# YxZhxn/Ray3D

Hardware: AMD Instinct MI355X
Metric: lifted poses/sec (17-joint, 243-frame window) (higher is better)
Workload: dtype f32; 1 GPU; BASELINE configs[1]: synthetic 17-joint 243-frame windows, batch 256 per GPU, forward-only pos+trj (C=256, latent 256, stage 3, camera embedding); batch_per_gpu=256, receptive_field=243, joints=17, parallelism=dp1 (independent window batches, no data-path collective), clock_settle_steps=60, world_size_observed=1

## Files before the change

### ray3d_amd/csrc/r3d_forward.cpp

```cpp
#include <algorithm>
#include <cstring>
#include <mutex>

#include "r3d_internal.hpp"
#include "r3d_undistort.hpp"

namespace r3d {

static void output_slots(int J, const int *first, int *slot) {
    int s = 0;
    auto put = [&](int part, int idx) {
        for (int f = 0; f < 3; ++f) slot[first[part] + idx * 3 + f] = s * 3 + f;
        ++s;
    };
    enum { T = 0, LA = 1, RA = 2, LL = 3, RL = 4 };
    if (J == 17) {
        put(T, 0);
        for (int i = 0; i < 3; ++i) put(LL, i);
        for (int i = 0; i < 3; ++i) put(RL, i);
        for (int i = 1; i < 5; ++i) put(T, i);
        for (int i = 0; i < 3; ++i) put(RA, i);
        for (int i = 0; i < 3; ++i) put(LA, i);
    } else if (J == 15) {
        put(T, 0); put(T, 1);
// ... 347 lines not shown
    hipError_t e;
    if ((e = c.rec.begin("r3d_event_pair", -1, 0, 0.0, 0.0)) != hipSuccess) return hip_fail(e, "hipEventRecord");
    if ((e = c.rec.end()) != hipSuccess) return hip_fail(e, "hipEventRecord");
    return R3D_OK;
}

int px_prepass(Call &c) {
    if (!c.in_px) return R3D_OK;
    const Model *a = c.a;
    const r3d_input *in_px = c.in_px;
    UndistArgs ua;
    memset(&ua, 0, sizeof ua);
    ua.uv = in_px->x_dev;
    ua.cam = in_px->cam_dev;
    ua.cam_stride = in_px->cam_stride;
    ua.rays = const_cast<float *>(c.in->x_dev);
    ua.J = a->cfg.num_joints;
    ua.npts = (int)(dist_ray_frames(a, in_px, c.B) * a->cfg.num_joints);
    ua.pts_per_window = dist_materialised(a, in_px) ? a->RF * a->cfg.num_joints : 0;
    ua.window_stride = (int)in_px->window_stride;
    ua.last_window = (int)(c.B - 1);
    ua.encoding = px_encoding(in_px->mode);
    if (const int rc = c.begin("r3d_undistort_rays_f64", (ua.npts + 255) / 256, 0.0, (double)ua.npts * (2 + enc_floats(ua.encoding)) * sizeof(float)); rc != R3D_OK)
        return rc;
    if (const hipError_t e = launch_undistort(ua, c.stream); e != hipSuccess) return hip_fail(e, "launch r3d_undistort_rays_f64");
    return c.end();
}

int pick_schedule(Call &c) {
    const Model *a = c.a, *b = c.b;
    const r3d_input *in = c.in;
    const Plan *pl = c.pl;
    c.uv = in->mode == R3D_INPUT_UV;
    c.JF = frame_floats(a, c.uv);
    c.bases.ws = reinterpret_cast<const char *>(c.ws);
    for (int mi = 0; mi < 2; ++mi)
        if (pl->m[mi]) {
            c.bases.arena[mi] = reinterpret_cast<const char *>(pl->m[mi]->d_arena);
            c.bases.iarena[mi] = reinterpret_cast<const char *>(pl->m[mi]->d_iarena);
        }
    c.bases.x = reinterpret_cast<const char *>(in->x_dev);
    c.bases.param = reinterpret_cast<const char *>(in->param_dev);
    c.bases.cam = reinterpret_cast<const char *>(in->cam_dev);
    c.shape.uv = c.uv;
    c.shape.window_stride = in->window_stride;
    c.shape.param_stride = in->param_stride;
    c.shape.cam_stride = in->cam_stride;
    c.shape.frames = c.frames;

    const FwdKeys keys = forward_keys(a, b);
    c.cu_limit = keys.cu_limit;
    c.sched = schedule_get(c.pl, c.B, keys.nwg, false, keys.lane_key0 + c.lane);
    if (!c.sched) return R3D_ERR_HIP;
    const Schedule *sched = c.sched;
    bool b3_call = false;
    for (const Model *mm : pl->m) b3_call = b3_call || (mm && mm->use_b3 && c.B >= b3_min_batch());
    c.shared = pl->frame_buf >= 0 && sched->d_frame_tiles != nullptr && in->window_stride == 1 && !b3_call &&
               (c.frames - 2) * 4 <= c.B * (int64_t)(a->RF / 3) && !(c.uv && in->cam_stride != 0) && !hook_on("R3D_NO_SHARED_L0") &&
               (unsigned long long)c.frames * (unsigned long long)pl->frame_ld * 4ull < 0xffffffffull;
    c.shape.shared = c.shared;
    c.variant = (c.uv ? 1 : 0) + (c.shared ? 2 : 0);
    c.single = forward_single_launch() && !a->opt_staged && !(b && b->opt_staged) && sched->fwd.grid > 0 && sched->fwd.d_rel[c.variant] != nullptr &&
               !(c.shared && sched->fwd.kernel != FWD_KERNEL_F32);
    return R3D_OK;
}

int frame_stage(Call &c) {
    if (!c.shared) return R3D_OK;
    const Plan *pl = c.pl;
    const r3d_input *in = c.in;
    const bool uv = c.uv;
    const StageSchedule &fs = c.sched->frame_stage;
    LaunchArgs la;
    memset(&la, 0, sizeof la);
    la.tiles = c.sched->d_frame_tiles;
    la.wg_off = c.sched->d_frame_wgoff;
    la.nprob = (int)pl->frame_probs.size();
    la.ks = fs.ks;
    float *fbase = reinterpret_cast<float *>(c.ws) + (size_t)pl->buffers[pl->frame_buf].offset_per_window * (size_t)c.B;
    for (int i = 0; i < la.nprob; ++i) {
        const Plan::FrameProb &f = pl->frame_probs[i];
        const Model *mm = pl->m[f.model];
        const Layer &L = mm->layers[f.layer];
        GemmProb &g = la.p[i];
        for (int sg = 0; sg < MAX_SEG; ++sg) g.kend[sg] = 0x7fffffff;
        g.w = mm->d_arena + L.w_off;
        g.bias = mm->d_arena + L.b_off;
        g.c = fbase + f.col;
        g.ldc = pl->frame_ld;
        g.M = (int)(c.frames - 2);
        g.N = L.N;
        g.K = L.Kpad;
        g.slope = 1.0f;
        g.lut = mm->d_iarena + (uv ? f.lut_uv : f.lut);
        g.x = reinterpret_cast<const float *>(in->x_dev);
        g.cam = uv ? reinterpret_cast<const double *>(in->cam_dev) : nullptr;
        g.cam_stride = 0;
        g.enc_ws = 0;
        g.enc_rows = g.M;
        g.enc_step = 1;
        g.enc_jf = c.JF;
        g.enc_cur = 0;
        g.enc_bytes = (unsigned)((size_t)c.frames * c.JF * sizeof(float));
        g.res_tap = 1;
    }
    if (const int rc = c.begin(uv ? "r3d_gemm_uv_f32" : "r3d_gemm_f32", fs.nwg, 0.0, 0.0); rc != R3D_OK) return rc;
    if (const hipError_t e = launch_gemm_stage(la, fs.nwg, STAGE_BIG, uv, c.stream); e != hipSuccess)
        return hip_fail(e, "launch r3d_gemm_f32 (per-frame first layers)");
    return c.end();
}


struct Single {
    hipStreamCaptureStatus cap = hipStreamCaptureStatusNone;
    bool own = false;
    bool poll = false;
    bool bound = false;
    char *ctrl = nullptr;
    size_t bank_bytes = 0;
    GemmProb *tables = nullptr;
    int bank = 0;
    unsigned *cnt = nullptr;
    BoundKey key;
};

void resolve_single(const Call &c, Single &s) {
    const Schedule::Fwd &fw = c.sched->fwd;
    const r3d_input *in = c.in;
    if (hipStreamIsCapturing(c.stream, &s.cap) != hipSuccess) { (void)hipGetLastError(); s.cap = hipStreamCaptureStatusActive; }
    s.own = s.cap == hipStreamCaptureStatusNone && fw.d_ctrl != nullptr;
    s.ctrl = s.own ? fw.d_ctrl : reinterpret_cast<char *>(c.ws) + workspace_act_bytes(c.pl, c.B);
    s.bank_bytes = ((size_t)(fw.ncnt + 4) * sizeof(unsigned) + 255) / 256 * 256;
    s.tables = reinterpret_cast<GemmProb *>(s.ctrl + (s.own ? 2 : 1) * s.bank_bytes);
    s.poll = s.own && fw.d_act != nullptr;
    s.key.variant = c.variant;
    s.key.base[BIND_WS] = c.ws;
    s.key.base[BIND_ARENA0] = c.bases.arena[0];
    s.key.base[BIND_ARENA1] = c.bases.arena[1];
    s.key.base[BIND_IARENA0] = c.bases.iarena[0];
    s.key.base[BIND_IARENA1] = c.bases.iarena[1];
    s.key.base[BIND_X] = in->x_dev;
    s.key.base[BIND_PARAM] = in->param_dev;
    s.key.base[BIND_CAM] = in->cam_dev;
    s.key.enc_ws = in->window_stride * c.JF;
    s.key.cam_stride = in->cam_stride;
    s.key.enc_bytes = (unsigned)((size_t)c.frames * c.JF * sizeof(float));
    s.key.param_stride = (int)in->param_stride;
    const Schedule::Fwd::Bound &bd = fw.bound;
    s.bound = s.own && bd.valid && bd.key == s.key;
    s.bank = s.bound ? bd.bank ^ 1 : 0;
    s.cnt = reinterpret_cast<unsigned *>(s.ctrl + (s.own ? s.bank : 0) * s.bank_bytes);
}

int bind_if_needed(Call &c, const Single &s) {
    if (s.bound) return R3D_OK;
    const Schedule::Fwd &fw = c.sched->fwd;
    BindArgs ba;
    memset(&ba, 0, sizeof ba);
    ba.rel = fw.d_rel[c.variant];
    ba.tags = fw.d_tags[c.variant];
    ba.out = s.tables;
    ba.nprob = fw.nprob;
    for (int k = 0; k < BIND_NBASE; ++k) ba.base[k] = s.key.base[k];
    ba.enc_ws = s.key.enc_ws;
    ba.cam_stride = s.key.cam_stride;
    ba.enc_bytes = s.key.enc_bytes;
    ba.param_stride = s.key.param_stride;
    ba.cnt = reinterpret_cast<unsigned *>(s.ctrl);
    ba.ncnt = s.own ? (int)(2 * s.bank_bytes / sizeof(unsigned)) - 4 : fw.ncnt;
    if (s.poll) {
        ba.base[BIND_WS] = fw.d_act;
        ba.arm = fw.d_act;
        ba.canon = 1;
        ba.arm_vec4 = (long long)(2 * fw.act_bytes / 16);
    }
    hipError_t e;
    if (const int rc = c.begin("r3d_bind_f32", 1, 0.0, 0.0); rc != R3D_OK) return rc;
    if ((e = launch_bind(ba, c.stream)) != hipSuccess) return hip_fail(e, "launch r3d_bind_f32");
    if (s.poll) {
        BindArgs b1 = ba;
        b1.base[BIND_WS] = fw.d_act + fw.act_bytes;
        b1.out = s.tables + fw.nprob;
        b1.ncnt = -4;
        b1.arm = nullptr;
        if ((e = launch_bind(b1, c.stream)) != hipSuccess) return hip_fail(e, "launch r3d_bind_f32");
    }
    return c.end();
}

int launch_tiles(Call &c, const Single &s, FwdArgs &fa) {
    Schedule::Fwd &fw = c.sched->fwd;
    const GemmProb *table = s.tables + (s.poll ? s.bank * fw.nprob : 0);
    if (s.poll) c.act_base = reinterpret_cast<float *>(fw.d_act + (size_t)s.bank * fw.act_bytes);
    fw.bound.valid = false;
    memset(&fa, 0, sizeof fa);
    fa.tiles = fw.d_tiles;
    fa.wg_off = fw.d_wgoff;
    fa.probs = table;
    fa.cnt = s.cnt;
    fa.cnt_next = s.own ? reinterpret_cast<unsigned *>(s.ctrl + (s.bank ^ 1) * s.bank_bytes) : nullptr;
    fa.ncnt = fw.ncnt;
    if (s.poll) {
        fa.poll = 1;
        fa.arm = fw.d_act + (size_t)(s.bank ^ 1) * fw.act_bytes;
        fa.arm_vec4 = (long long)(fw.act_bytes / 16);
    }
    fa.spin_ticks = (long long)std::max(c.a->spin_timeout_ms, 1) * 100000LL;
    if (const char *ft = hook_env("R3D_FAULT_TILE")) fa.fault_tile1 = atoi(ft) + 1;
    const bool uv_launch = c.uv && fw.uses_gather;
    const int fwd_kernel = c.shared ? FWD_KERNEL_CLIP : fw.kernel;
    if (const int rc = c.begin(forward_kernel_name(fwd_kernel, uv_launch), fw.grid, fw.flops, fw.bytes); rc != R3D_OK) return rc;
#ifdef R3D_TIMING
    timing_arm_forward(fw, fa, c.stream);
#endif
    if (const hipError_t e = launch_forward(fa, fw.grid, fwd_kernel, uv_launch, c.stream); e != hipSuccess) return hip_fail(e, "launch r3d_forward_f32");
    c.a->last_clk_dev = s.cap == hipStreamCaptureStatusNone ? s.cnt + fw.ncnt + 2 : nullptr;
    return R3D_OK;
}

int launch_in_order(Call &c, const Single &s, FwdArgs &fa) {
    Model *a = c.a;
    hipError_t e;
    std::lock_guard<std::mutex> launch_lock(g_fwd_launch_mu);
    if ((e = order_single_launch(c.stream, true, c.cu_limit > 0)) != hipSuccess) return hip_fail(e, "hipStreamWaitEvent");
    if (c.cu_limit > 0 && a->lanes <= 1 && a->last_fwd_stream && a->last_fwd_stream != c.stream) {
        if ((e = wait_behind(c.stream, (hipStream_t)a->last_fwd_stream, a->order_ev)) != hipSuccess) return hip_fail(e, "hipStreamWaitEvent");
    }
    a->last_fwd_stream = c.stream;
    if (const int rc = bind_if_needed(c, s); rc != R3D_OK) return rc;
    if (const int rc = launch_tiles(c, s, fa); rc != R3D_OK) return rc;
    if ((e = order_single_launch(c.stream, false, c.cu_limit > 0)) != hipSuccess) return hip_fail(e, "hipEventRecord");
    return R3D_OK;
}

int single_launch(Call &c) {
    Schedule::Fwd &fw = c.sched->fwd;
    Single s;
    resolve_single(c, s);
    FwdArgs fa;
    if (const int rc = launch_in_order(c, s, fa); rc != R3D_OK) return rc;
    if (s.own) {
        fw.bound.valid = true;
        fw.bound.bank = s.bank;
        fw.bound.key = s.key;
    }
#ifdef R3D_TIMING
    timing_report_forward(c.pl, fw, fa, c.B, c.stream);
#endif
    if (const int rc = c.end(); rc != R3D_OK) return rc;
    c.abort_flag = s.cnt + fw.ncnt;
    return R3D_OK;
}

int staged_level(Call &c, size_t si) {
    const Plan *pl = c.pl;
    const auto &st = (*c.sched->levels)[si];
    const StageSchedule &ss = c.sched->stages[si];
    LaunchArgs la;
    memset(&la, 0, sizeof la);
    la.tiles = c.sched->d_tiles + ss.tiles_off;
    la.wg_off = c.sched->d_wgoff + ss.wgoff_off;
    la.nprob = (int)st.size();
    la.ks = ss.ks;
    int n_enc = 0;
    for (int i = 0; i < la.nprob; ++i) {
        const ProbSpec &q = pl->probs[st[i] & ~STAGE_SPILL_IN];
        if (q.enc_lut >= 0 && q.enc_kernel) ++n_enc;
        const int rc = fill_prob(pl, q, c.B, c.a, c.bases, c.shape, la.p[i], nullptr);
        if (rc != R3D_OK) return rc;
    }
    if (n_enc != 0 && n_enc != la.nprob) { set_error("internal: launch mixes encoded and plain operands"); return R3D_ERR_STATE; }
    if ((n_enc != 0) != (ss.kind == STAGE_ENC)) { set_error("internal: schedule and plan disagree on the launch kind"); return R3D_ERR_STATE; }
    bool uv_launch = false;
    for (int i = 0; i < la.nprob; ++i) uv_launch = uv_launch || la.p[i].cam != nullptr;
    bool b3_launch = false;
    for (int i = 0; i < la.nprob; ++i) b3_launch = b3_launch || la.p[i].wb3 != nullptr;
    const char *kname = ss.kind == STAGE_ENC ? (uv_launch ? "r3d_gemm_enc_uv_f32" : "r3d_gemm_enc_f32")
                      : b3_launch ? (uv_launch ? "r3d_gemm_uv_b3" : "r3d_gemm_b3") : (uv_launch ? "r3d_gemm_uv_f32" : "r3d_gemm_f32");
    if (const int rc = c.begin(kname, ss.nwg, ss.flops, ss.bytes); rc != R3D_OK) return rc;
#ifdef R3D_TIMING
    const bool timed = timing_arm_stage(si, la, c.stream);
#endif
    if (const hipError_t e = launch_gemm_stage(la, ss.nwg, ss.kind, uv_launch, c.stream); e != hipSuccess) return hip_fail(e, "launch r3d_gemm_f32");
#ifdef R3D_TIMING
    if (timed) timing_report_stage(si, ss, c.stream);
#endif
    return c.end();
}

int staged_levels(Call &c) {
    c.a->last_clk_dev = nullptr;
    for (size_t si = 0; si < c.sched->levels->size(); ++si)
        if (const int rc = staged_level(c, si); rc != R3D_OK) return rc;
    return R3D_OK;
}

int decoder_tail(Call &c) {
    const Model *a = c.a;
    const Plan *pl = c.pl;
    auto buf_ptr = [&](int id) -> float * { return c.act_base + (size_t)pl->buffers[id].offset_per_window * (size_t)c.B; };
    DecodeArgs da;
    memset(&da, 0, sizeof da);
    da.B = c.B;
    da.J = a->cfg.num_joints;
    da.has_pos = pl->pos_model >= 0;
    da.has_trj = pl->trj_model >= 0;
    da.out = c.out;
    da.out_trj = da.has_pos ? c.out_trj : nullptr;
    da.abort_flag = c.abort_flag;
    da.status = a->status_host;
    double dec_flops = 0;
    int first = 0;
    std::vector<Plan::Dec> order;
    for (const auto &d : pl->decs) if (pl->m[d.model]->cfg.kind == R3D_KIND_POS) order.push_back(d);
    for (const auto &d : pl->decs) if (pl->m[d.model]->cfg.kind == R3D_KIND_TRJ) order.push_back(d);
    int firsts[MAX_DEC] = {0};
    for (const auto &d : order) {
        const Model *m = pl->m[d.model];
        const Layer &L = m->layers[d.layer];
        const int sidx = da.nsrc++;
        da.h[sidx] = buf_ptr(d.hbuf);
        da.w[sidx] = m->d_arena + L.w_off;
        da.bias[sidx] = m->d_arena + L.b_off;
        da.n_out[sidx] = L.N;
        da.first[sidx] = first;
        firsts[sidx] = first;
        if (m->cfg.kind == R3D_KIND_POS) first += L.N;
        dec_flops += 2.0 * (double)c.B * L.K * L.N;
    }
    if (da.has_pos) output_slots(da.J, firsts, da.slot);
    if (const int rc = c.begin(c.B >= 128 ? "r3d_decode_w4_f32" : "r3d_decode_f32", 0, dec_flops, (double)c.B * da.nsrc * MLP_HIDDEN * 4.0); rc != R3D_OK) return rc;
    if (const hipError_t e = launch_decode(da, c.stream); e != hipSuccess) return hip_fail(e, "launch r3d_decode_f32");
    if (const int rc = c.end(); rc != R3D_OK) return rc;
    if (c.rec.on()) c.a->nrec = (int)c.rec.n;
    return R3D_OK;
}

int relay_done(Call &c) {
    Model::Lane *relay = c.relay;
    if (!relay) return R3D_OK;
    if (const hipError_t e = hipEventRecord(relay->done, relay->stream); e != hipSuccess) return hip_fail(e, "hipEventRecord(lane)");
    if (std::find(relay->waiters.begin(), relay->waiters.end(), c.caller_stream) == relay->waiters.end()) relay->waiters.push_back(c.caller_stream);
    return R3D_OK;
}

}

int forward_run(Model *a, Model *b, const r3d_input *in, int64_t B, float *out, float *out_trj, void *ws, size_t ws_bytes,
                void *stream) {
    Call c{a, b, in, B, out, out_trj, ws, ws_bytes, stream, (hipStream_t)stream};
    int rc = check_call(c);
    if (rc == R3D_OK) rc = redirect_px(c);
    if (rc == R3D_OK) rc = pick_plan(c);
    if (rc == R3D_OK) rc = pick_lane(c);
    if (rc == R3D_OK) rc = empty_bracket(c);
    if (rc == R3D_OK) rc = px_prepass(c);
    if (rc == R3D_OK) rc = pick_schedule(c);
    if (rc == R3D_OK) rc = frame_stage(c);
    if (rc == R3D_OK) rc = c.single ? single_launch(c) : staged_levels(c);
    if (rc == R3D_OK) rc = decoder_tail(c);
    if (rc == R3D_OK) rc = relay_done(c);
    return rc;
}

}
```

### ray3d_amd/csrc/r3d_internal.hpp

```cpp
#pragma once

#include <hip/hip_runtime.h>

#include <cstdint>
#include <cstdlib>
#include <map>
#include <mutex>
#include <string>
#include <vector>

#include "ray3d_hip.h"

namespace r3d {

constexpr int BK = 32;
constexpr int MAX_SEG = 4;
constexpr int MAX_PROB = 12;
constexpr int N_ALIGN = 256;
constexpr int MLP_HIDDEN = 1024;
constexpr int EMBED_MID = 32;
constexpr int CUR_LD = 64;


struct GemmProb {
    const float *a[MAX_SEG];
    int lda[MAX_SEG];
    int kend[MAX_SEG];
    const float *w;
    const float *bias;
    const float *res;
    float *c;
    int ldr, ldc;
    int M, N, K;
    float slope;
    const float *w2;
    const float *bias2;
    int K2;
    float slope2;
    const float *wb3;
    const float *w2b3, *w3b3;
    const float *w3;
    const float *bias3;
    int K3;
    float slope3;
    const int *lut;
    const float *x;
    long long enc_ws;
    int enc_rows;
    int enc_jf;
    int enc_cur;
    int enc_step;
    unsigned enc_bytes;
    int res_tap;
    int canon;
    const double *cam;
    long long cam_stride;
};

struct LaunchArgs {
    const int4 *tiles;
    const int *wg_off;
    int nprob;
    int ks;
    long long *dbg;
    GemmProb p[MAX_PROB];
};

constexpr int FWD_TILE_INT4 = 6;
constexpr int FWD_MAX_DEP = 8;
struct FwdArgs {
    const int4 *tiles;
    const int *wg_off;
    const GemmProb *probs;
    unsigned *cnt;
    unsigned *cnt_next;
    int ncnt;
    int poll;
    void *arm;
    long long arm_vec4;
    long long spin_ticks;
    int fault_tile1;
    long long *dbg;
};
enum { FWD_KERNEL_F32 = 0, FWD_KERNEL_B3 = 1, FWD_KERNEL_LAT = 2, FWD_KERNEL_CLIP = 3, FWD_KERNEL_COUNT = 4 };
constexpr int BIND_NPTR = 18;
enum { BIND_NULL = 0, BIND_WS, BIND_ARENA0, BIND_ARENA1, BIND_IARENA0, BIND_IARENA1, BIND_X, BIND_PARAM, BIND_CAM, BIND_NBASE };
struct BindArgs {
    const GemmProb *rel;
    const unsigned char *tags;
    GemmProb *out;
    unsigned *cnt;
    int nprob, ncnt;
    const void *base[BIND_NBASE];
    long long enc_ws, cam_stride;
    unsigned enc_bytes;
    int param_stride;
    int canon;
    void *arm;
    long long arm_vec4;
};

struct UndistArgs {
    const float *uv;
    const double *cam;
    long long cam_stride;
    float *rays;
    int npts;
    int J;
    int pts_per_window;
    int window_stride;
    int last_window;
    int encoding;
};

struct ClipsEncArgs {
    const r3d_clip_input_desc *table;
    const float *px;
    float *x;
    float *x_mirror;
    int32_t *status;
    long long total_frames, out_rows, max_rows;
    unsigned long long mirror_inv[2];
    int J;
    int encoding;
};

constexpr int MAX_DEC = 6;
struct DecodeArgs {
    const float *h[MAX_DEC];
    const float *w[MAX_DEC];
    const float *bias[MAX_DEC];
    int n_out[MAX_DEC];
    int first[MAX_DEC];
    int nsrc;
    int has_pos, has_trj;
    int J;
    long long B;
    float *out;
    float *out_trj;
    const unsigned *abort_flag;
    unsigned *status;
    int slot[5 * 16];
};


struct TensorSpec {
    std::string key;
    int rank;
    int64_t shape[4];
    int64_t numel() const {
        int64_t n = 1;
        for (int i = 0; i < rank; ++i) n *= shape[i];
        return n;
    }
};

inline int64_t b3_min_batch() {
    return 96;
}

inline bool env_on(const char *name) {
    const char *e = getenv(name);
    return e && atoi(e) != 0;
}
#ifdef R3D_TEST_HOOKS
inline bool hook_on(const char *name) { return env_on(name); }
inline const char *hook_env(const char *name) { return getenv(name); }
#else
inline bool hook_on(const char *) { return false; }
inline const char *hook_env(const char *) { return nullptr; }
#endif

struct Layer {
    std::string weight_key;
    std::string bias_key;
    std::string bn_prefix;
    int taps;
    int cin;
    int N, K, Npad, Kpad;
    float slope;
    std::vector<int> colmap;
    std::vector<int> colmap_neg;
    bool frag;
    size_t w_off, b_off;
    bool bf3 = false;
    bool bf3_conv = false;
    size_t wb3_off = 0;
    struct Pre { int ref_col0, ref_width, new_width, shrink_layer; };
    std::vector<Pre> pre;
    int cin_ref = 0;
    int shared_of = -1;
    int shared_split = 0;
};

struct Model {
    r3d_config cfg;
    int RF;
    std::vector<TensorSpec> specs;
    std::map<std::string, int> spec_index;
    std::vector<std::vector<float>> host_weights;
    std::vector<bool> have;
    std::vector<Layer> layers;
    std::map<std::string, int> layer_index;
    struct Branch {
        std::string prefix;
        std::vector<int> joints;
        int cin, k0, k0pad;
        size_t lut_off;
        size_t lut_uv_off;
        size_t lut_frame_off = 0, lut_frame_uv_off = 0;
        int frame_layer = -1;
    };
    std::vector<Branch> branches;
    size_t global_lut_off = 0;
    size_t global_lut_uv_off = 0;
    bool use_b3 = false;
    bool fold_shrink = false;
    std::vector<float> arena;
    std::vector<int> iarena;
    float *d_arena = nullptr;
    int *d_iarena = nullptr;
    int device = -1;
    bool finalized = false;
    bool dirty = true;
    bool opt_staged = false;
    int spin_timeout_ms = 1000;
    int cu_limit = 0;
    void *last_fwd_stream = nullptr;
    hipEvent_t order_ev = nullptr;
    int lanes = 0;
    struct Lane {
        hipStream_t stream = nullptr;
        hipEvent_t done = nullptr, in = nullptr;
        std::vector<void *> waiters;
    };
    Lane lane[4];
    int next_lane = 0;
    const unsigned *last_clk_dev = nullptr;
    unsigned *status_host = nullptr;
    bool profiling = false;
    struct Rec {
        hipEvent_t e0, e1;
        r3d_launch_record r;
    };
    std::vector<Rec> recs;
    int nrec = 0;
    uint64_t id = 0;
    ~Model();
};

struct BufferSpec {
    std::string name;
    int64_t floats_per_window;
    int external;
    int64_t offset_per_window;
};

struct ProbSpec {
    int model;
    int layer;
    int rows_per_window;
    int nseg;
    struct Seg { int buf, col, ld, width; } seg[MAX_SEG];
    int res_buf, res_col, res_ld;
    int c_buf, c_col, c_ld;
    int layer2;
    int layer3;
    int enc_lut;
    int enc_lut_uv;
    bool enc_kernel;
    int enc_rows;
    int enc_step;
    int frame_col = -1;
    std::vector<int> deps;
    int depth;
    double flops_per_window;
};

struct StageSchedule {
    int nwg;
    int ks;
    int kind;
    int ntiles;
    size_t tiles_off;
    size_t wgoff_off;
    double flops, bytes;
    double imbalance;
    double makespan;
};

struct BoundKey {
    int variant = 0;
    const void *base[BIND_NBASE] = {nullptr};
    long long enc_ws = 0, cam_stride = 0;
    unsigned enc_bytes = 0;
    int param_stride = 0;
    bool operator==(const BoundKey &o) const {
        bool same = variant == o.variant && enc_ws == o.enc_ws && cam_stride == o.cam_stride && enc_bytes == o.enc_bytes &&
                    param_stride == o.param_stride;
        for (int k = 0; same && k < BIND_NBASE; ++k) same = base[k] == o.base[k];
        return same;
    }
};

struct Schedule {
    int64_t B = 0;
    bool pinned = false;
    int spill_row0 = -1;
    const std::vector<std::vector<int>> *levels = nullptr;
    std::vector<StageSchedule> stages;
    int4 *d_tiles = nullptr;
    int *d_wgoff = nullptr;
    StageSchedule frame_stage{};
    int4 *d_frame_tiles = nullptr;
    int *d_frame_wgoff = nullptr;
    struct Fwd {
        int grid = 0, ntiles = 0, ncnt = 0, nprob = 0;
        std::vector<int> cnt_base;
        int4 *d_tiles = nullptr;
        int *d_wgoff = nullptr;
        GemmProb *d_rel[4] = {nullptr, nullptr, nullptr, nullptr};
        unsigned char *d_tags[4] = {nullptr, nullptr, nullptr, nullptr};
        std::vector<int> h_tiles, h_wgoff;
        double flops = 0, bytes = 0;
        bool uses_gather = false;
        int kernel = FWD_KERNEL_F32;
        char *d_ctrl = nullptr;
        size_t bank_bytes = 0;
        char *d_act = nullptr;
        size_t act_bytes = 0;
        struct Bound {
            bool valid = false;
            int bank = 0;
            BoundKey key;
        } bound;
    } fwd;
    ~Schedule();
};

struct Plan {
    const Model *m[2] = {nullptr, nullptr};
    std::vector<BufferSpec> buffers;
    std::vector<ProbSpec> probs;
    std::vector<std::vector<int>> stages;
    std::vector<std::vector<int>> stages_spill;
    std::vector<std::vector<int>> stages_spill_alt;
    std::vector<std::vector<int>> stages_asap;
    int spill_prob = -1;
    int kind = 0;
    int64_t floats_per_window = 0;
    int64_t tail_floats = 0;
    int frame_buf = -1, frame_ld = 0;
    struct FrameProb { int model, layer, col, lut, lut_uv; };
    std::vector<FrameProb> frame_probs;
    int emb_buf[2] = {-1, -1};
    int param_buf = -1;
    struct Dec { int model, layer, hbuf; };
    std::vector<Dec> decs;
    int pos_model = -1, trj_model = -1;
    std::map<int64_t, Schedule *> schedules;
    std::vector<int64_t> schedule_lru;
    ~Plan();
};

struct Bases {
    const char *ws = nullptr, *arena[2] = {nullptr, nullptr}, *iarena[2] = {nullptr, nullptr};
    const char *x = nullptr, *param = nullptr, *cam = nullptr;
};
struct CallShape {
    bool uv = false;
    bool shared = false;
    int64_t window_stride = 0, param_stride = 0, cam_stride = 0;
    long long frames = 0;
};

inline int frame_floats(const Model *a, bool uv) { return a->cfg.num_joints * (uv ? 2 : a->cfg.in_features); }

struct ModelPair { Model *a, *b; };
inline ModelPair model_pair(const r3d_model *pos, const r3d_model *trj) {
    Model *p = const_cast<Model *>(reinterpret_cast<const Model *>(pos)), *t = const_cast<Model *>(reinterpret_cast<const Model *>(trj));
    return {p ? p : t, p ? t : nullptr};
}

int fill_prob(const Plan *pl, const ProbSpec &q, int64_t B, const Model *a, const Bases &bs, const CallShape &cs, GemmProb &g,
              unsigned char *tags);
bool same_input_shape(const Model *a, const Model *b);
size_t workspace_bytes_pair(Model *a, Model *b, int64_t B);
int dist_check(const Model *a, const r3d_input *in, bool need_cam);
size_t dist_ray_bytes(const Model *a, const r3d_input *in, int64_t B);
struct FwdKeys { int cu_limit, nwg, lane_key0, nlanes; };
FwdKeys forward_keys(const Model *a, const Model *b);
int forward_run(Model *a, Model *b, const r3d_input *in, int64_t B, float *out, float *out_trj, void *ws, size_t ws_bytes, void *stream);

extern std::mutex g_fwd_launch_mu;
hipError_t wait_behind(hipStream_t stream, hipStream_t other, hipEvent_t &ev);
hipError_t order_single_launch(hipStream_t stream, bool before, bool masked = false);
int lanes_create(Model *m, int n);
void lanes_destroy(Model *m);

int valid_check_args(const char *what, const float *pos, const float *trj, const float *gt, int64_t n, int32_t J,
                     const int32_t *parents, int32_t flags, const double *out);

int clips_encode_check_args(const char *what, const float *px, int64_t total_frames, int32_t J, int32_t encoding,
                            const r3d_clip_input_desc *clips, int32_t num_clips, int64_t max_rows, const float *x, int64_t out_rows,
                            const float *x_mirror, const int32_t *mirror_perm, const int32_t *status);

#ifdef R3D_TIMING
void timing_arm_forward(const Schedule::Fwd &fw, FwdArgs &fa, hipStream_t stream);
void timing_report_forward(const Plan *pl, const Schedule::Fwd &fw, const FwdArgs &fa, int64_t B, hipStream_t stream);
bool timing_arm_stage(size_t si, LaunchArgs &la, hipStream_t stream);
void timing_report_stage(size_t si, const StageSchedule &ss, hipStream_t stream);
#endif

void set_error(const char *fmt, ...);
const char *last_error();
int hip_fail(hipError_t e, const char *what);

Model *model_create(const r3d_config &cfg);
int model_set_weight(Model *m, const char *key, const float *host, const int64_t *shape, int rank);
int model_finalize(Model *m);
enum { PLAN_FUSED = 0, PLAN_SMALL = 1, PLAN_MEDIUM = 2, PLAN_LARGE = 3 };
int plan_kind(int64_t B);
std::vector<int64_t> plan_kind_edges();
Plan *plan_get(Model *a, Model *b, int kind);
void plans_drop(const Model *m);
bool plans_pinned(const Model *m);
constexpr int STAGE_SPILL_IN = 1 << 30;
constexpr int GEMM_SCHED_MAX_UNITS = 6;
struct SchedProb {
    int M, N, nk;
    int max_ks;
    int max_units;
    int nk2 = 0;
    int row0 = 0;
    bool gemv = false;
    bool lat = false;
    bool nb_ok = false;
};
constexpr int GEMV_ROWS = 4;
constexpr int COL_GRANULE = 32;
constexpr int NB_CODE = 64;
constexpr bool tile_is_nb(int ks) { return ks > NB_CODE; }
constexpr bool tile_is_narrow(int ks) { return ks >= 8 && ks < NB_CODE; }
constexpr int tile_width(int ks) { return ks > NB_CODE ? (ks - NB_CODE) * 32 : ks >= 8 ? 32 : 256 / ks; }
void schedule_stage(const std::vector<SchedProb> &probs, int nwg, int max_units, std::vector<int4> &tiles,
                    std::vector<int> &wgoff, StageSchedule &out, bool enc = false);
inline size_t frag_index(int o, int k, int nk) {
    const int nb = o >> 5, li = o & 31, kt = k >> 5, kin = k & 31, lh = kin >> 4, q = (kin & 15) >> 2, e = kin & 3;
    return ((((size_t)nb * nk + kt) * 4 + q) * 64 + (lh * 32 + li)) * 4 + e;
}
const std::vector<std::vector<int>> *schedule_build_host(const Plan *pl, int64_t B, int nwg, int &spill_row0, std::vector<int4> &tiles,
                                                        std::vector<int> &wgoff, std::vector<StageSchedule> &stages);
bool schedule_build_fwd(const Plan *pl, int64_t B, int nwg, const std::vector<std::vector<int>> &levels, const std::vector<StageSchedule> &stages,
                        const std::vector<int4> &tiles, const std::vector<int> &wgoff, Schedule::Fwd &fw, std::vector<int> &out_tiles,
                        std::vector<int> &out_wgoff);
Schedule *schedule_get(Plan *pl, int64_t B, int nwg, bool pin = false, int lane = 0);
inline int64_t schedule_key(int64_t B, int lane) { return B | ((int64_t)lane << 48); }
int device_cu_count();

enum { STAGE_BIG = 0, STAGE_ENC = 1 };
typedef void (*GemmKernel)(const LaunchArgs);
typedef void (*FwdKernel)(const FwdArgs);
GemmKernel gemm_kernel_f32(bool uv);
GemmKernel gemm_kernel_enc(bool uv);
GemmKernel gemm_kernel_b3(bool uv);
FwdKernel fwd_kernel_f32(bool uv);
FwdKernel fwd_kernel_b3(bool uv);
FwdKernel fwd_kernel_lat(bool uv);
FwdKernel fwd_kernel_clip(bool uv);
hipError_t launch_gemm_stage(const LaunchArgs &args, int nwg, int kind, bool uv, hipStream_t stream);
hipError_t launch_decode(const DecodeArgs &args, hipStream_t stream);
hipError_t launch_forward(const FwdArgs &args, int nwg, int kind, bool uv, hipStream_t stream);
const char *forward_kernel_name(int kind, bool uv);
int forward_resident_capacity(int kind, bool uv);
hipError_t launch_bind(const BindArgs &args, hipStream_t stream);
hipError_t launch_undistort(const UndistArgs &args, hipStream_t stream);
hipError_t launch_clips_encode(const ClipsEncArgs &args, int num_clips, hipStream_t stream);
bool forward_single_launch();
size_t fwd_ctrl_bytes(const Plan *pl, int64_t B);

inline int round_up(int v, int m) { return (v + m - 1) / m * m; }

constexpr int ENC_INVALID = (int)0x80000000u;

int launch_clip_metrics(const float *pred, const float *gt, long long n, int J, const double *Rn2w, const double *Tn2w,
                        double *out, double *frame, double *detail, hipStream_t stream);
int launch_clip_valid(const float *pos, const float *trj, const float *gt, long long n, int J, const int32_t *parents,
                      int flags, double *out, double *frame, hipStream_t stream);
size_t clips_metrics_scratch_bytes(int num_clips, long long max_frames, bool detail);
int launch_clips_metrics(const float *pred, const float *gt, long long total, int J, const r3d_clip_desc *table, int num_clips,
                         long long max_frames, double *rows, long long row_stride, double *detail, long long detail_stride,
                         double *frame, void *scratch, hipStream_t stream);

}
```

### ray3d_amd/csrc/r3d_kernels.hip

```cpp
#include "r3d_tiles.hpp"

namespace r3d {

extern "C" __global__ __launch_bounds__(256) void r3d_bind_f32(const BindArgs b) {
    const int i = blockIdx.x * blockDim.x + threadIdx.x, total = gridDim.x * blockDim.x;
    for (int j = i; j < b.ncnt + 4; j += total) b.cnt[j] = 0u;
    if (b.arm != nullptr) {
        typedef unsigned u32x4 __attribute__((ext_vector_type(4)));
        const u32x4 sv = {ACT_SENTINEL, ACT_SENTINEL, ACT_SENTINEL, ACT_SENTINEL};
        for (long long j = i; j < b.arm_vec4; j += total) reinterpret_cast<u32x4 *>(b.arm)[j] = sv;
    }
    if (i >= b.nprob) return;
    GemmProb g = b.rel[i];
    const unsigned char *tg = b.tags + (size_t)i * BIND_NPTR;
    auto fix = [&](auto &ptr, int k) {
        const int tag = tg[k];
        typedef typename std::remove_reference<decltype(ptr)>::type PT;
        ptr = tag == BIND_NULL ? (PT) nullptr : (PT)((const char *)b.base[tag] + (size_t)ptr);
    };
    for (int sgi = 0; sgi < MAX_SEG; ++sgi) {
        if (tg[sgi] == BIND_PARAM) g.lda[sgi] = b.param_stride;
        fix(g.a[sgi], sgi);
    }
    fix(g.w, 4); fix(g.bias, 5); fix(g.res, 6); fix(g.c, 7); fix(g.w2, 8); fix(g.bias2, 9); fix(g.wb3, 10); fix(g.w2b3, 11);
    fix(g.w3b3, 12); fix(g.w3, 13); fix(g.bias3, 14); fix(g.lut, 15); fix(g.x, 16); fix(g.cam, 17);
    g.canon = b.canon;
    if (g.lut != nullptr) {
        g.enc_ws = b.enc_ws;
        g.enc_bytes = b.enc_bytes;
        g.cam_stride = b.cam_stride;
    }
    b.out[i] = g;
}


hipError_t launch_gemm_stage(const LaunchArgs &args, int nwg, int kind, bool uv, hipStream_t stream) {
    bool b3 = false;
    for (int i = 0; i < args.nprob; ++i) b3 = b3 || args.p[i].wb3 != nullptr;
    static bool attr_done_dev[64] = {false};
    int dev = 0;
    if (hipGetDevice(&dev) != hipSuccess || dev < 0 || dev >= 64) dev = 0;
    bool &attr_done = attr_done_dev[dev];
    if (!attr_done) {
        for (int u = 0; u < 2; ++u) {
            hipError_t e = hipFuncSetAttribute(reinterpret_cast<const void *>(gemm_kernel_f32(u != 0)), hipFuncAttributeMaxDynamicSharedMemorySize, GEMM_LDS_BYTES);
            if (e != hipSuccess) return e;
            if ((e = hipFuncSetAttribute(reinterpret_cast<const void *>(gemm_kernel_b3(u != 0)), hipFuncAttributeMaxDynamicSharedMemorySize, GEMM_LDS_BYTES)) != hipSuccess) return e;
            if ((e = hipFuncSetAttribute(reinterpret_cast<const void *>(gemm_kernel_enc(u != 0)), hipFuncAttributeMaxDynamicSharedMemorySize, ENC_LDS_BYTES)) != hipSuccess) return e;
        }
        attr_done = true;
    }
    if (kind == STAGE_ENC) gemm_kernel_enc(uv)<<<dim3(nwg), dim3(GEMM_THREADS), ENC_LDS_BYTES, stream>>>(args);
    else (b3 ? gemm_kernel_b3(uv) : gemm_kernel_f32(uv))<<<dim3(nwg), dim3(GEMM_THREADS), GEMM_LDS_BYTES, stream>>>(args);
    return hipGetLastError();
}

static FwdKernel forward_kernel(int kind, bool uv) {
    switch (kind) {
        case FWD_KERNEL_B3: return fwd_kernel_b3(uv);
        case FWD_KERNEL_LAT: return fwd_kernel_lat(uv);
        case FWD_KERNEL_CLIP: return fwd_kernel_clip(uv);
        default: return fwd_kernel_f32(uv);
    }
}
const char *forward_kernel_name(int kind, bool uv) {
    switch (kind) {
        case FWD_KERNEL_B3: return uv ? "r3d_forward_uv_b3" : "r3d_forward_b3";
        case FWD_KERNEL_LAT: return uv ? "r3d_forward_uv_lat" : "r3d_forward_lat";
        case FWD_KERNEL_CLIP: return uv ? "r3d_forward_clip_uv_f32" : "r3d_forward_clip_f32";
        default: return uv ? "r3d_forward_uv_f32" : "r3d_forward_f32";
    }
}

static hipError_t forward_set_lds_attr() {
    static bool attr_done_dev[64] = {false};
    int dev = 0;
    if (hipGetDevice(&dev) != hipSuccess || dev < 0 || dev >= 64) dev = 0;
    if (!attr_done_dev[dev]) {
        for (int k = 0; k < FWD_KERNEL_COUNT; ++k)
            for (int u = 0; u < 2; ++u) {
                hipError_t e = hipFuncSetAttribute(reinterpret_cast<const void *>(forward_kernel(k, u != 0)), hipFuncAttributeMaxDynamicSharedMemorySize, GEMM_LDS_BYTES);
                if (e != hipSuccess) return e;
            }
        attr_done_dev[dev] = true;
    }
    return hipSuccess;
}

hipError_t launch_forward(const FwdArgs &args, int nwg, int kind, bool uv, hipStream_t stream) {
    if (hipError_t e = forward_set_lds_attr(); e != hipSuccess) return e;
    forward_kernel(kind, uv)<<<dim3(nwg), dim3(GEMM_THREADS), GEMM_LDS_BYTES, stream>>>(args);
    return hipGetLastError();
}

int forward_resident_capacity(int kind, bool uv) {
    int per_cu = 0;
    if (forward_set_lds_attr() != hipSuccess ||
        hipOccupancyMaxActiveBlocksPerMultiprocessor(&per_cu, reinterpret_cast<const void *>(forward_kernel(kind, uv)), GEMM_THREADS, GEMM_LDS_BYTES) != hipSuccess) {
        (void)hipGetLastError();
        return 0;
    }
    return per_cu * device_cu_count();
}

hipError_t launch_bind(const BindArgs &args, hipStream_t stream) {
    const int threads = std::max(args.nprob, std::min((int)std::max<long long>(args.ncnt + 4, args.arm ? args.arm_vec4 : 0), 256 * 256));
    r3d_bind_f32<<<dim3((threads + 255) / 256), dim3(256), 0, stream>>>(args);
    return hipGetLastError();
}


template <int CTRL, int ROW_MASK>
__device__ __forceinline__ float dpp_add(float x) {
    return x + __builtin_bit_cast(float, __builtin_amdgcn_update_dpp(0, __builtin_bit_cast(int, x), CTRL, ROW_MASK, 0xf, false));
}
__device__ __forceinline__ float wave_sum(float v) {
    v = dpp_add<0xb1, 0xf>(v);
    v = dpp_add<0x4e, 0xf>(v);
    v = dpp_add<0x141, 0xf>(v);
    v = dpp_add<0x140, 0xf>(v);
    v = dpp_add<0x142, 0xa>(v);
    v = dpp_add<0x143, 0xc>(v);
    return __builtin_bit_cast(float, __builtin_amdgcn_readlane(__builtin_bit_cast(int, v), 63));
}

struct DecodeJoint {
    f32x4 w[3][4];
    __device__ __forceinline__ void load(const float *wrows, int lane) {
#pragma unroll
        for (int n = 0; n < 3; ++n)
#pragma unroll
            for (int j = 0; j < 4; ++j) w[n][j] = gload4(wrows + (size_t)n * MLP_HIDDEN + j * 256 + lane * 4);
    }
    __device__ __forceinline__ void dot(const f32x4 (&hv)[4], float (&o)[3]) const {
#pragma unroll
        for (int n = 0; n < 3; ++n) {
            float acc = 0.0f;
#pragma unroll
            for (int j = 0; j < 4; ++j)
                acc += hv[j][0] * w[n][j][0] + hv[j][1] * w[n][j][1] + hv[j][2] * w[n][j][2] + hv[j][3] * w[n][j][3];
            o[n] = wave_sum(acc);
        }
    }
};

template <int DECODE_WINDOWS>
__device__ __forceinline__ void decode_body(const DecodeArgs &a) {
    const int lane = threadIdx.x & 63;
    const long long gw = (long long)blockIdx.x * 4 + (threadIdx.x >> 6);
    const int per_win = a.has_pos ? a.J : 1;
    const long long b0 = gw / per_win * DECODE_WINDOWS;
    if (b0 >= a.B) return;
    const bool poisoned = a.abort_flag != nullptr && __hip_atomic_load((gu32)a.abort_flag, __ATOMIC_RELAXED, __HIP_MEMORY_SCOPE_AGENT) != 0;
    const float poison = poisoned ? __builtin_nanf("") : 0.0f;
    if (poisoned && a.status != nullptr && gw == 0 && lane == 0) __hip_atomic_store((gu32)a.status, 1u, __ATOMIC_RELAXED, __HIP_MEMORY_SCOPE_SYSTEM);
    const int jf = (int)(gw % per_win);
    const int ts = a.nsrc - 1;
    int s = 0, o = 0;
    if (a.has_pos) {
        const int npos = a.has_trj ? a.nsrc - 1 : a.nsrc;
        for (int q = 0; q < npos; ++q)
            if (3 * jf >= a.first[q]) { s = q; o = 3 * jf - a.first[q]; }
    }
    f32x4 hv[2][4], ht[2][4];
    DecodeJoint rt, rj;
    if (a.has_trj) rt.load(a.w[ts], lane);
    if (a.has_pos) rj.load(a.w[s] + (size_t)o * MLP_HIDDEN, lane);
    auto load_window = [&](int i) {
        const long long b = b0 + i < a.B ? b0 + i : a.B - 1;
        if (a.has_trj) {
#pragma unroll
            for (int j = 0; j < 4; ++j) ht[i & 1][j] = gload4(a.h[ts] + b * MLP_HIDDEN + j * 256 + lane * 4);
        }
        if (a.has_pos) {
#pragma unroll
            for (int j = 0; j < 4; ++j) hv[i & 1][j] = gload4(a.h[s] + b * MLP_HIDDEN + j * 256 + lane * 4);
        }
    };
    load_window(0);
    float bt[3] = {0.0f, 0.0f, 0.0f}, bj[3] = {0.0f, 0.0f, 0.0f};
    int e = 0;
    if (a.has_trj) {
#pragma unroll
        for (int n = 0; n < 3; ++n) bt[n] = a.bias[ts][n];
    }
    if (a.has_pos) {
        e = a.slot[a.first[s] + o];
#pragma unroll
        for (int n = 0; n < 3; ++n) bj[n] = a.bias[s][o + n];
    }
#pragma unroll
    for (int i = 0; i < DECODE_WINDOWS; ++i) {
        if (i + 1 < DECODE_WINDOWS) load_window(i + 1);
        const long long b = b0 + i;
        const bool live = b < a.B;
        float trj[3] = {0.0f, 0.0f, 0.0f};
        if (a.has_trj) {
            rt.dot(ht[i & 1], trj);
#pragma unroll
            for (int n = 0; n < 3; ++n) trj[n] += bt[n] + poison;
            if (live && lane == 0 && jf == 0) {
#pragma unroll
                for (int n = 0; n < 3; ++n) {
                    if (a.out_trj) a.out_trj[b * 3 + n] = trj[n];
                    if (!a.has_pos) a.out[b * 3 + n] = trj[n];
                }
            }
        }
        if (!a.has_pos) continue;
        float v[3];
        rj.dot(hv[i & 1], v);
        if (live && lane == 0) {
#pragma unroll
            for (int n = 0; n < 3; ++n) a.out[b * (a.J * 3) + e + n] = v[n] + bj[n] + trj[n] + poison;
        }
    }
}

extern "C" __global__ __launch_bounds__(256) void r3d_decode_f32(const DecodeArgs a) { decode_body<1>(a); }
extern "C" __global__ __launch_bounds__(256) void r3d_decode_w4_f32(const DecodeArgs a) { decode_body<4>(a); }

hipError_t launch_decode(const DecodeArgs &args, hipStream_t stream) {
    const int w = args.B >= 128 ? 4 : 1;
    const long long waves = (args.B + w - 1) / w * (args.has_pos ? args.J : 1);
    if (w == 4) r3d_decode_w4_f32<<<dim3((unsigned)((waves + 3) / 4)), dim3(256), 0, stream>>>(args);
    else r3d_decode_f32<<<dim3((unsigned)((waves + 3) / 4)), dim3(256), 0, stream>>>(args);
    return hipGetLastError();
}

}
```

Baseline: 455,700 poses/s.

## Restructure decode to per-source waves over window groups with batched reductions

The large-batch decode kernel now launches one workgroup per group of windows, with one wave per decoder source. Each wave loads its hidden rows once and iterates over its joints with double-buffered weight fetches. Results go to shared memory and are combined with the trajectory in a final cooperative store. Wave reductions are batched across outputs so the DPP steps interleave, and windows-per-group is picked from the CU count. This trades re-reading hidden vectors per joint for re-reading weights per group, and adds a sync plus serial per-joint loops within each wave.

```diff
diff --git a/ray3d_amd/csrc/r3d_forward.cpp b/ray3d_amd/csrc/r3d_forward.cpp
--- a/ray3d_amd/csrc/r3d_forward.cpp
+++ b/ray3d_amd/csrc/r3d_forward.cpp
@@ -673,6 +673,7 @@
     DecodeArgs da;
     memset(&da, 0, sizeof da);
     da.B = c.B;
+    da.wpg = decode_windows_per_group(c.B);
     da.J = a->cfg.num_joints;
     da.has_pos = pl->pos_model >= 0;
     da.has_trj = pl->trj_model >= 0;
@@ -700,7 +701,7 @@
         dec_flops += 2.0 * (double)c.B * L.K * L.N;
     }
     if (da.has_pos) output_slots(da.J, firsts, da.slot);
-    if (const int rc = c.begin(c.B >= 128 ? "r3d_decode_w4_f32" : "r3d_decode_f32", 0, dec_flops, (double)c.B * da.nsrc * MLP_HIDDEN * 4.0); rc != R3D_OK) return rc;
+    if (const int rc = c.begin(da.wpg > 0 ? "r3d_decode_w4_f32" : "r3d_decode_f32", 0, dec_flops, (double)c.B * da.nsrc * MLP_HIDDEN * 4.0); rc != R3D_OK) return rc;
     if (const hipError_t e = launch_decode(da, c.stream); e != hipSuccess) return hip_fail(e, "launch r3d_decode_f32");
     if (const int rc = c.end(); rc != R3D_OK) return rc;
     if (c.rec.on()) c.a->nrec = (int)c.rec.n;
diff --git a/ray3d_amd/csrc/r3d_internal.hpp b/ray3d_amd/csrc/r3d_internal.hpp
--- a/ray3d_amd/csrc/r3d_internal.hpp
+++ b/ray3d_amd/csrc/r3d_internal.hpp
@@ -136,6 +136,7 @@
     int has_pos, has_trj;
     int J;
     long long B;
+    int wpg;
     float *out;
     float *out_trj;
     const unsigned *abort_flag;
@@ -469,6 +470,7 @@
 FwdKernel fwd_kernel_lat(bool uv);
 FwdKernel fwd_kernel_clip(bool uv);
 hipError_t launch_gemm_stage(const LaunchArgs &args, int nwg, int kind, bool uv, hipStream_t stream);
+int decode_windows_per_group(long long B);
 hipError_t launch_decode(const DecodeArgs &args, hipStream_t stream);
 hipError_t launch_forward(const FwdArgs &args, int nwg, int kind, bool uv, hipStream_t stream);
 const char *forward_kernel_name(int kind, bool uv);
diff --git a/ray3d_amd/csrc/r3d_kernels.hip b/ray3d_amd/csrc/r3d_kernels.hip
--- a/ray3d_amd/csrc/r3d_kernels.hip
+++ b/ray3d_amd/csrc/r3d_kernels.hip
@@ -114,15 +114,33 @@
 __device__ __forceinline__ float dpp_add(float x) {
     return x + __builtin_bit_cast(float, __builtin_amdgcn_update_dpp(0, __builtin_bit_cast(int, x), CTRL, ROW_MASK, 0xf, false));
 }
-__device__ __forceinline__ float wave_sum(float v) {
-    v = dpp_add<0xb1, 0xf>(v);
-    v = dpp_add<0x4e, 0xf>(v);
-    v = dpp_add<0x141, 0xf>(v);
-    v = dpp_add<0x140, 0xf>(v);
-    v = dpp_add<0x142, 0xa>(v);
-    v = dpp_add<0x143, 0xc>(v);
-    return __builtin_bit_cast(float, __builtin_amdgcn_readlane(__builtin_bit_cast(int, v), 63));
-}
+template <int N>
+__device__ __forceinline__ void wave_sums(float (&v)[N]) {
+#pragma unroll
+    for (int i = 0; i < N; ++i) v[i] = dpp_add<0xb1, 0xf>(v[i]);
+#pragma unroll
+    for (int i = 0; i < N; ++i) v[i] = dpp_add<0x4e, 0xf>(v[i]);
+#pragma unroll
+    for (int i = 0; i < N; ++i) v[i] = dpp_add<0x141, 0xf>(v[i]);
+#pragma unroll
+    for (int i = 0; i < N; ++i) v[i] = dpp_add<0x140, 0xf>(v[i]);
+#pragma unroll
+    for (int i = 0; i < N; ++i) v[i] = dpp_add<0x142, 0xa>(v[i]);
+#pragma unroll
+    for (int i = 0; i < N; ++i) v[i] = dpp_add<0x143, 0xc>(v[i]);
+#pragma unroll
+    for (int i = 0; i < N; ++i) v[i] = __builtin_bit_cast(float, __builtin_amdgcn_readlane(__builtin_bit_cast(int, v[i]), 63));
+}
+__device__ __forceinline__ float decode_partial(const f32x4 (&hv)[4], const f32x4 (&w)[4]) {
+    float acc = 0.0f;
+#pragma unroll
+    for (int j = 0; j < 4; ++j)
+        acc += hv[j][0] * w[j][0] + hv[j][1] * w[j][1] + hv[j][2] * w[j][2] + hv[j][3] * w[j][3];
+    return acc;
+}
+__device__ __forceinline__ float decode_trj(float sum, float bias, float poison) { return sum + (bias + poison); }
+__device__ __forceinline__ float decode_pre(float sum, float bias) { return sum + bias; }
+__device__ __forceinline__ float decode_pose(float pre, float trj, float poison) { return pre + trj + poison; }
 
 struct DecodeJoint {
     f32x4 w[3][4];
@@ -132,28 +150,29 @@
 #pragma unroll
             for (int j = 0; j < 4; ++j) w[n][j] = gload4(wrows + (size_t)n * MLP_HIDDEN + j * 256 + lane * 4);
     }
-    __device__ __forceinline__ void dot(const f32x4 (&hv)[4], float (&o)[3]) const {
-#pragma unroll
-        for (int n = 0; n < 3; ++n) {
-            float acc = 0.0f;
-#pragma unroll
-            for (int j = 0; j < 4; ++j)
-                acc += hv[j][0] * w[n][j][0] + hv[j][1] * w[n][j][1] + hv[j][2] * w[n][j][2] + hv[j][3] * w[n][j][3];
-            o[n] = wave_sum(acc);
-        }
+    template <int NW>
+    __device__ __forceinline__ void dot(const f32x4 (&hv)[NW][4], float (&o)[NW * 3]) const {
+#pragma unroll
+        for (int i = 0; i < NW; ++i)
+#pragma unroll
+            for (int n = 0; n < 3; ++n) o[i * 3 + n] = decode_partial(hv[i], w[n]);
+        wave_sums<NW * 3>(o);
     }
 };
 
-template <int DECODE_WINDOWS>
+__device__ __forceinline__ float decode_poison(const DecodeArgs &a, bool first_lane) {
+    const bool poisoned = a.abort_flag != nullptr && __hip_atomic_load((gu32)a.abort_flag, __ATOMIC_RELAXED, __HIP_MEMORY_SCOPE_AGENT) != 0;
+    if (poisoned && a.status != nullptr && first_lane) __hip_atomic_store((gu32)a.status, 1u, __ATOMIC_RELAXED, __HIP_MEMORY_SCOPE_SYSTEM);
+    return poisoned ? __builtin_nanf("") : 0.0f;
+}
+
 __device__ __forceinline__ void decode_body(const DecodeArgs &a) {
     const int lane = threadIdx.x & 63;
     const long long gw = (long long)blockIdx.x * 4 + (threadIdx.x >> 6);
     const int per_win = a.has_pos ? a.J : 1;
-    const long long b0 = gw / per_win * DECODE_WINDOWS;
-    if (b0 >= a.B) return;
-    const bool poisoned = a.abort_flag != nullptr && __hip_atomic_load((gu32)a.abort_flag, __ATOMIC_RELAXED, __HIP_MEMORY_SCOPE_AGENT) != 0;
-    const float poison = poisoned ? __builtin_nanf("") : 0.0f;
-    if (poisoned && a.status != nullptr && gw == 0 && lane == 0) __hip_atomic_store((gu32)a.status, 1u, __ATOMIC_RELAXED, __HIP_MEMORY_SCOPE_SYSTEM);
+    const long long b = gw / per_win;
+    if (b >= a.B) return;
+    const float poison = decode_poison(a, gw == 0 && lane == 0);
     const int jf = (int)(gw % per_win);
     const int ts = a.nsrc - 1;
     int s = 0, o = 0;
@@ -162,22 +181,18 @@
         for (int q = 0; q < npos; ++q)
             if (3 * jf >= a.first[q]) { s = q; o = 3 * jf - a.first[q]; }
     }
-    f32x4 hv[2][4], ht[2][4];
+    f32x4 hv[1][4], ht[1][4];
     DecodeJoint rt, rj;
     if (a.has_trj) rt.load(a.w[ts], lane);
     if (a.has_pos) rj.load(a.w[s] + (size_t)o * MLP_HIDDEN, lane);
-    auto load_window = [&](int i) {
-        const long long b = b0 + i < a.B ? b0 + i : a.B - 1;
-        if (a.has_trj) {
-#pragma unroll
-            for (int j = 0; j < 4; ++j) ht[i & 1][j] = gload4(a.h[ts] + b * MLP_HIDDEN + j * 256 + lane * 4);
-        }
-        if (a.has_pos) {
-#pragma unroll
-            for (int j = 0; j < 4; ++j) hv[i & 1][j] = gload4(a.h[s] + b * MLP_HIDDEN + j * 256 + lane * 4);
-        }
-    };
-    load_window(0);
+    if (a.has_trj) {
+#pragma unroll
+        for (int j = 0; j < 4; ++j) ht[0][j] = gload4(a.h[ts] + b * MLP_HIDDEN + j * 256 + lane * 4);
+    }
+    if (a.has_pos) {
+#pragma unroll
+        for (int j = 0; j < 4; ++j) hv[0][j] = gload4(a.h[s] + b * MLP_HIDDEN + j * 256 + lane * 4);
+    }
     float bt[3] = {0.0f, 0.0f, 0.0f}, bj[3] = {0.0f, 0.0f, 0.0f};
     int e = 0;
     if (a.has_trj) {
@@ -189,42 +204,120 @@
 #pragma unroll
         for (int n = 0; n < 3; ++n) bj[n] = a.bias[s][o + n];
     }
-#pragma unroll
-    for (int i = 0; i < DECODE_WINDOWS; ++i) {
-        if (i + 1 < DECODE_WINDOWS) load_window(i + 1);
-        const long long b = b0 + i;
-        const bool live = b < a.B;
-        float trj[3] = {0.0f, 0.0f, 0.0f};
-        if (a.has_trj) {
-            rt.dot(ht[i & 1], trj);
-#pragma unroll
-            for (int n = 0; n < 3; ++n) trj[n] += bt[n] + poison;
-            if (live && lane == 0 && jf == 0) {
-#pragma unroll
-                for (int n = 0; n < 3; ++n) {
-                    if (a.out_trj) a.out_trj[b * 3 + n] = trj[n];
-                    if (!a.has_pos) a.out[b * 3 + n] = trj[n];
-                }
+    float trj[3] = {0.0f, 0.0f, 0.0f};
+    if (a.has_trj) {
+        rt.dot<1>(ht, trj);
+#pragma unroll
+        for (int n = 0; n < 3; ++n) trj[n] = decode_trj(trj[n], bt[n], poison);
+        if (lane == 0 && jf == 0) {
+#pragma unroll
+            for (int n = 0; n < 3; ++n) {
+                if (a.out_trj) a.out_trj[b * 3 + n] = trj[n];
+                if (!a.has_pos) a.out[b * 3 + n] = trj[n];
             }
         }
-        if (!a.has_pos) continue;
-        float v[3];
-        rj.dot(hv[i & 1], v);
-        if (live && lane == 0) {
-#pragma unroll
-            for (int n = 0; n < 3; ++n) a.out[b * (a.J * 3) + e + n] = v[n] + bj[n] + trj[n] + poison;
+    }
+    if (!a.has_pos) return;
+    float v[3];
+    rj.dot<1>(hv, v);
+    if (lane == 0) {
+#pragma unroll
+        for (int n = 0; n < 3; ++n) a.out[b * (a.J * 3) + e + n] = decode_pose(decode_pre(v[n], bj[n]), trj[n], poison);
+    }
+}
+
+constexpr int DECODE_MAX_WPG = 4;
+constexpr int DECODE_MAX_OUT = 5 * 16;
+template <int WPG>
+__device__ __forceinline__ void decode_group(const DecodeArgs &a, float *sh_pre, float *sh_trj) {
+    const int lane = threadIdx.x & 63;
+    const int s = __builtin_amdgcn_readfirstlane(threadIdx.x >> 6);
+    const long long b0 = (long long)blockIdx.x * WPG;
+    const float poison = decode_poison(a, blockIdx.x == 0 && threadIdx.x == 0);
+    const bool is_trj = a.has_trj && s == a.nsrc - 1;
+    const int J3 = a.J * 3;
+    const float *wsrc = a.w[s], *bsrc = a.bias[s];
+    const int nj = a.n_out[s] / 3;
+    f32x4 hv[WPG][4];
+#pragma unroll
+    for (int i = 0; i < WPG; ++i) {
+        const long long b = b0 + i < a.B ? b0 + i : a.B - 1;
+#pragma unroll
+        for (int j = 0; j < 4; ++j) hv[i][j] = gload4(a.h[s] + b * MLP_HIDDEN + j * 256 + lane * 4);
+    }
+    auto joint = [&](const DecodeJoint &r, const float (&bias)[3], int e) {
+        float v[WPG * 3];
+        r.template dot<WPG>(hv, v);
+        if (lane != 0) return;
+        if (!is_trj) {
+#pragma unroll
+            for (int i = 0; i < WPG; ++i)
+#pragma unroll
+                for (int n = 0; n < 3; ++n) sh_pre[i * DECODE_MAX_OUT + e + n] = decode_pre(v[i * 3 + n], bias[n]);
+            return;
         }
-    }
-}
-
-extern "C" __global__ __launch_bounds__(256) void r3d_decode_f32(const DecodeArgs a) { decode_body<1>(a); }
-extern "C" __global__ __launch_bounds__(256) void r3d_decode_w4_f32(const DecodeArgs a) { decode_body<4>(a); }
+#pragma unroll
+        for (int i = 0; i < WPG; ++i) {
+            float t[3];
+#pragma unroll
+            for (int n = 0; n < 3; ++n) sh_trj[i * 3 + n] = t[n] = decode_trj(v[i * 3 + n], bias[n], poison);
+            if (b0 + i >= a.B) continue;
+            float *dst = a.has_pos ? a.out_trj : a.out;
+            if (dst == nullptr) continue;
+#pragma unroll
+            for (int n = 0; n < 3; ++n) dst[(b0 + i) * 3 + n] = t[n];
+        }
+    };
+    auto fetch = [&](DecodeJoint &r, int q, float (&bias)[3], int &e) {
+        r.load(wsrc + (size_t)q * 3 * MLP_HIDDEN, lane);
+#pragma unroll
+        for (int n = 0; n < 3; ++n) bias[n] = bsrc[q * 3 + n];
+        e = is_trj ? 0 : a.slot[a.first[s] + q * 3];
+    };
+    DecodeJoint r0, r1;
+    float c0[3], c1[3];
+    int e0 = 0, e1 = 0;
+    fetch(r0, 0, c0, e0);
+    for (int q = 0; q < nj; q += 2) {
+        if (q + 1 < nj) fetch(r1, q + 1, c1, e1);
+        joint(r0, c0, e0);
+        if (q + 1 >= nj) break;
+        if (q + 2 < nj) fetch(r0, q + 2, c0, e0);
+        joint(r1, c1, e1);
+    }
+    if (!a.has_pos) return;
+    __syncthreads();
+    for (int t = threadIdx.x; t < WPG * J3; t += blockDim.x) {
+        const int i = t / J3, k = t - i * J3;
+        if (b0 + i >= a.B) break;
+        const float trj = a.has_trj ? sh_trj[i * 3 + k % 3] : 0.0f;
+        a.out[(b0 + i) * J3 + k] = decode_pose(sh_pre[i * DECODE_MAX_OUT + k], trj, poison);
+    }
+}
+
+extern "C" __global__ __launch_bounds__(256) void r3d_decode_f32(const DecodeArgs a) { decode_body(a); }
+extern "C" __global__ __launch_bounds__(64 * MAX_DEC) void r3d_decode_w4_f32(const DecodeArgs a) {
+    __shared__ float sh_pre[DECODE_MAX_WPG * DECODE_MAX_OUT], sh_trj[DECODE_MAX_WPG * 3];
+    if (a.wpg == 4) decode_group<4>(a, sh_pre, sh_trj);
+    else if (a.wpg == 2) decode_group<2>(a, sh_pre, sh_trj);
+    else decode_group<1>(a, sh_pre, sh_trj);
+}
+
+int decode_windows_per_group(long long B) {
+    if (B < 128) return 0;
+    const long long cus = std::max(device_cu_count(), 1);
+    for (int wpg = 1; wpg < DECODE_MAX_WPG; wpg *= 2)
+        if ((B + wpg - 1) / wpg <= cus) return wpg;
+    return DECODE_MAX_WPG;
+}
 
 hipError_t launch_decode(const DecodeArgs &args, hipStream_t stream) {
-    const int w = args.B >= 128 ? 4 : 1;
-    const long long waves = (args.B + w - 1) / w * (args.has_pos ? args.J : 1);
-    if (w == 4) r3d_decode_w4_f32<<<dim3((unsigned)((waves + 3) / 4)), dim3(256), 0, stream>>>(args);
-    else r3d_decode_f32<<<dim3((unsigned)((waves + 3) / 4)), dim3(256), 0, stream>>>(args);
+    if (args.wpg > 0) {
+        r3d_decode_w4_f32<<<dim3((unsigned)((args.B + args.wpg - 1) / args.wpg)), dim3(64 * args.nsrc), 0, stream>>>(args);
+    } else {
+        const long long waves = args.B * (args.has_pos ? args.J : 1);
+        r3d_decode_f32<<<dim3((unsigned)((waves + 3) / 4)), dim3(256), 0, stream>>>(args);
+    }
     return hipGetLastError();
 }
 
```

Result: no change. 457,400 poses/s (median of 6 runs) (+0.4%).
